# Sudo42b/vision.cpp

Hardware: AMD Instinct MI355X
Metric: images/sec, Depth-Anything-V2-Small 518x518 f16 (higher is better)
Workload: dtype f16

## Files before the change

vision.cpp_amd/csrc/kernels_dconv.hip:

```cpp
#include "vx_common.h"

#include <cmath>
#include <cstdlib>
#include <type_traits>

namespace {

typedef __attribute__((address_space(1))) const void* gptr_t;
typedef __attribute__((address_space(3))) void* lptr_t;

constexpr int TRASH_BLOCKS = 1024;
__device__ __attribute__((aligned(16))) unsigned char g_dconv_trash[TRASH_BLOCKS * 8 * 1024];

constexpr int DCONV_TAB_MAX = 1280;
constexpr int CK = 32;
constexpr int PIXB = CK * 2;
constexpr int NW = 8;

struct tile_grid {
    int ncols, nrows, n_main, n_strip, strip_x0;
    __host__ __device__ tile_grid(int H, int W) {
        const int q = W / 32, rem = W % 32;
        const bool strip = rem > 0 && rem <= 16;
        ncols = q + ((rem > 16) ? 1 : 0);
        nrows = (H + 15) / 16;
        n_main = ncols * nrows;
        n_strip = strip ? (H + 31) / 32 : 0;
        strip_x0 = q * 32;
    }
    __host__ __device__ int total() const { return n_main + n_strip; }
};

__device__ __forceinline__ float relu1(float x) { return __int_as_float(max(__float_as_int(x), 0)); }

template <int COUT, int EPI, bool AR, bool STAMP, int RES = 0, int HSV = (COUT == 32 ? 3 : 2), bool BIL = false, bool ONE = false>
__global__ __launch_bounds__(512) void dconv3x3_kernel(const vx_dconv_args p) {
    static_assert(!ONE || COUT == 32, "single-step tiles: COUT = 32 only");
    constexpr int MT = 2;
    constexpr int HALO_PIX = 18 * 34;
    constexpr int HJ = 5, HALO_INSTR = HJ * NW, HALO_BYTES = HALO_INSTR * 1024;
    constexpr int NI = COUT / 32;
    constexpr int W_BYTES = 9 * COUT * PIXB, W_INSTR = W_BYTES / 1024;
    constexpr int WJ = (W_INSTR + NW - 1) / NW;
    constexpr int HS = HSV;
    constexpr int WSLOTS = RES ? RES : 2;
    static_assert(!RES || COUT == 32, "resident slabs are built for COUT = 32 (the COUT = 64 epilogue stages through slab space)");
    static_assert(!BIL || (COUT == 32 && HSV == 2 && !RES && !AR), "the interpolating loader is built for COUT = 32 with two halo stages");
    constexpr int SRC_PIX = 256, SRC_BYTES = SRC_PIX * PIXB, SJ = SRC_BYTES / 1024 / NW;
    constexpr int SRC_BASE = HS * HALO_BYTES;
    constexpr int W_BASE = HS * HALO_BYTES + (BIL ? 2 * SRC_BYTES : 0);
    constexpr int BIAS_BASE = W_BASE + WSLOTS * W_BYTES;
    constexpr int TAB_BASE = BIAS_BASE + ((COUT * 4 + 15) & ~15);
    static_assert(!BIL || TAB_BASE + (DCONV_TAB_MAX + 4) * 8 <= 160 * 1024, "interpolation tables do not fit");
    constexpr int NCH16 = COUT / 8, PITCH = COUT * 2;
    static_assert(BIAS_BASE + COUT * 4 <= 160 * 1024, "LDS ring too large");
    static_assert(256 * PITCH <= HALO_BYTES && 256 * PITCH <= W_BYTES + (COUT == 32 ? HALO_BYTES : 0), "output staging does not fit a stage");

    extern __shared__ __attribute__((aligned(16))) unsigned char smem[];
    float* const s_bias = reinterpret_cast<float*>(smem + BIAS_BASE);

    const int tid = threadIdx.x, lane = tid & 63;
    const int wave = __builtin_amdgcn_readfirstlane(tid >> 6);
    const int r = lane & 31, h = lane >> 5;
    const int H = p.H, W = p.W;
    const tile_grid tg(H, W);
    const int per_image = tg.total();
    const int total = p.B * per_image;

    int t_cur, t_end, t_step;
    {
        const int id = blockIdx.x, xcd = id & 7;
        const int per = total >> 3, rem = total & 7;
        const int lo = xcd < rem ? xcd * (per + 1) : rem * (per + 1) + (xcd - rem) * per;
        t_end = lo + per + (xcd < rem ? 1 : 0);
        t_step = ((int)gridDim.x - xcd + 7) >> 3;
        t_cur = lo + (id >> 3);
    }
    if (t_cur >= t_end) return;

    if (tid < COUT) s_bias[tid] = p.bias ? p.bias[tid] : 0.0f;

    const int up = p.up2 ? 1 : 0;
    const int Hs = BIL ? p.bil_hs : H >> up, Ws = BIL ? p.bil_ws : W >> up;
    const int nch = p.cin / CK;
    const int nch_total_bytes = nch * 9 * COUT * PIXB;
    const long x_plane_bytes = p.x_plane * 2;
    const int x_pix = p.x_pix ? (int)p.x_pix : CK;
    const long out_pix = p.out_pix ? p.out_pix : CK, res1_pix = p.res1_pix ? p.res1_pix : CK, res2_pix = p.res2_pix ? p.res2_pix : CK;

    uint2* const tab_y = reinterpret_cast<uint2*>(smem + TAB_BASE);
    uint2* const tab_x = tab_y + H + 2;
    if constexpr (BIL) {
        const float sfy = (H > 1 && Hs > 1) ? (float)(H - 1) / (float)(Hs - 1) : (float)H / (float)Hs;
        const float sfx = (W > 1 && Ws > 1) ? (float)(W - 1) / (float)(Ws - 1) : (float)W / (float)Ws;
        for (int i = tid; i < H + W + 4; i += 512) {
            const bool isx = i >= H + 2;
            const int o = (isx ? i - (H + 2) : i) - 1, n_out = isx ? W : H, n_src = isx ? Ws : Hs;
            uint2 e = {0x80000000u, 0u};
            if (o >= 0 && o < n_out) {
                const float sc = (float)o / (isx ? sfx : sfy);
                int i0 = (int)floorf(sc);
                i0 = max(0, min(i0, n_src - 1));
                const float f = fminf(fmaxf(sc - (float)i0, 0.0f), 1.0f);
                e.x = (i0 + 1 < n_src ? 0x40000000u : 0u) | (unsigned)i0 << 16;
                e.y = (unsigned)__builtin_bit_cast(unsigned short, (f16)(1.0f - f)) | (unsigned)__builtin_bit_cast(unsigned short, (f16)f) << 16;
            }
            tab_y[i] = e;
        }
        __syncthreads();
    }

    struct geom { int b, y0, x0, tws; };
    auto locate = [&](int t) {
        geom g;
        g.b = t / per_image;
        const int k = t - g.b * per_image;
        if (k < tg.n_main) {
            const int ty = k / tg.ncols;
            g.y0 = ty * 16; g.x0 = (k - ty * tg.ncols) * 32; g.tws = 5;
        } else {
            g.y0 = (k - tg.n_main) * 32; g.x0 = tg.strip_x0; g.tws = 4;
        }
        return g;
    };
    constexpr unsigned OOB = 0x80000000u;
    unsigned hoff[HJ];
    unsigned hpack[HJ];
    auto setup_shape_src = [&](int tws) {
        const int hw = (1 << tws) + 2;
#pragma unroll
        for (int j = 0; j < HJ; ++j) {
            const int L = (wave + j * NW) * 64 + lane;
            const int pix = L >> 2, phys = L & 3;
            const int hy = tws == 5 ? pix / 34 : pix / 18;
            const int hx = pix - hy * hw;
            hpack[j] = (unsigned)(pix < HALO_PIX ? hy : 255) | (unsigned)hx << 8 | (unsigned)(phys ^ ((pix >> 2) & 3)) << 16 | (pix < HALO_PIX ? 1u << 24 : 0u);
        }
    };
    __amdgpu_buffer_rsrc_t x_rsrc;
    const __amdgpu_buffer_rsrc_t w_rsrc = __builtin_amdgcn_make_buffer_rsrc(const_cast<void*>(p.w), 0, nch_total_bytes, 0x00020000);
    auto setup_src = [&](const geom& g) {
        const long img_bytes = (long)Hs * Ws * x_pix * 2;
        const long span = x_pix > CK ? img_bytes : (nch - 1) * x_plane_bytes + img_bytes;
        x_rsrc = __builtin_amdgcn_make_buffer_rsrc(const_cast<char*>(reinterpret_cast<const char*>(p.x)) + g.b * img_bytes, 0, (int)span, 0x00020000);
#pragma unroll
        for (int j = 0; j < HJ; ++j) {
            unsigned pk = hpack[j];
            asm volatile("" : "+v"(pk));
            const int iy = g.y0 - 1 + (int)(pk & 0xff), ix = g.x0 - 1 + (int)((pk >> 8) & 0xff);
            const bool valid = (pk >> 24) && (unsigned)iy < (unsigned)H && (unsigned)ix < (unsigned)W;
            const int e = ((iy >> up) * Ws + (ix >> up)) * x_pix + (int)(((pk >> 16) & 3) << 3);
            hoff[j] = valid ? (unsigned)(e * 2) : OOB;
        }
    };
    unsigned spack[SJ];
    unsigned soff[SJ];
    auto patch_w = [](int tws) { return tws == 5 ? 21 : 12; };
    auto setup_shape_patch = [&](int tws) {
        const int pw = patch_w(tws);
#pragma unroll
        for (int j = 0; j < SJ; ++j) {
            const int L = (wave + j * NW) * 64 + lane, q = L >> 2;
            const int prow = q / pw;
            spack[j] = (unsigned)prow | (unsigned)(q - prow * pw) << 8 | (unsigned)(L & 3) << 16 | (q < 252 ? 1u << 24 : 0u);
        }
    };
    auto patch_origin = [&](int y0, int x0, int& py0, int& px0) {
        py0 = (__builtin_amdgcn_readfirstlane(tab_y[max(y0 - 1, 0) + 1].x) >> 16) & 0x3fff;
        px0 = (__builtin_amdgcn_readfirstlane(tab_x[max(x0 - 1, 0) + 1].x) >> 16) & 0x3fff;
    };
    auto setup_patch = [&](const geom& g) {
        const long img_bytes = (long)Hs * Ws * x_pix * 2;
        const long span = x_pix > CK ? img_bytes : (nch - 1) * x_plane_bytes + img_bytes;
        x_rsrc = __builtin_amdgcn_make_buffer_rsrc(const_cast<char*>(reinterpret_cast<const char*>(p.x)) + g.b * img_bytes, 0, (int)span, 0x00020000);
        int py0, px0;
        patch_origin(g.y0, g.x0, py0, px0);
#pragma unroll
        for (int j = 0; j < SJ; ++j) {
            unsigned pk = spack[j];
            asm volatile("" : "+v"(pk));
            const int sy = py0 + (int)(pk & 0xff), sx = px0 + (int)((pk >> 8) & 0xff);
            const bool valid = (pk >> 24) && sy < Hs && sx < Ws;
            soff[j] = valid ? (unsigned)(((sy * Ws + sx) * x_pix + (int)(((pk >> 16) & 3) << 3)) * 2) : OOB;
        }
    };
    auto issue_patch = [&](int c, int sstage) {
#pragma unroll
        for (int j = 0; j < SJ; ++j)
            __builtin_amdgcn_raw_ptr_buffer_load_lds(x_rsrc, (lptr_t)(smem + SRC_BASE + sstage * SRC_BYTES + (wave + j * NW) * 1024), 16, soff[j],
                                                     c * (int)x_plane_bytes, 0, 0);
    };
    unsigned ioff[HJ], ifr[HJ];
    unsigned short idy[HJ];
    int i_shape = -1;
    auto setup_interp = [&](const geom& g) {
        if (g.tws != i_shape) {
            i_shape = g.tws;
            setup_shape_src(i_shape);
        }
        int py0, px0;
        patch_origin(g.y0, g.x0, py0, px0);
        const int pw = patch_w(g.tws), org = py0 * pw + px0;
#pragma unroll
        for (int j = 0; j < HJ; ++j) {
            unsigned pk = hpack[j];
            asm volatile("" : "+v"(pk));
            const uint2 ty = tab_y[min(g.y0 + (int)(pk & 0xff), H + 1)], tx = tab_x[min(g.x0 + (int)((pk >> 8) & 0xff), W + 1)];
            const bool outside = (int)(ty.x | tx.x) < 0;
            const int sy = (ty.x >> 16) & 0x3fff, sx = (tx.x >> 16) & 0x3fff;
            const unsigned lg16 = ((pk >> 16) & 3) * 16;
            const unsigned o00 = (outside ? 252u * PIXB : (unsigned)((sy * pw + sx - org) * PIXB)) + lg16;
            ioff[j] = o00 | (o00 + (outside ? 0u : ((tx.x >> 30) & 1) * PIXB)) << 16;
            idy[j] = (unsigned short)(outside ? 0u : ((ty.x >> 30) & 1) * (unsigned)(pw * PIXB));
            ifr[j] = (tx.y >> 16) | (ty.y & 0xffff0000u);
        }
    };
    typedef _Float16 h2 __attribute__((ext_vector_type(2)));
    auto lerp2 = [](h2 v, h2 w, h2 f) { return f * w + (v - f * v); };
    auto interp_unit = [&](int j, int sstage, int hstage) {
        const unsigned char* const sp = smem + SRC_BASE + sstage * SRC_BYTES;
        const unsigned o0 = ioff[j] & 0xffffu, o1 = ioff[j] >> 16, dy = idy[j];
        const f16x8 a = *reinterpret_cast<const f16x8*>(sp + o0), b = *reinterpret_cast<const f16x8*>(sp + o1);
        const f16x8 c = *reinterpret_cast<const f16x8*>(sp + o0 + dy), d = *reinterpret_cast<const f16x8*>(sp + o1 + dy);
        const h2 fr = __builtin_bit_cast(h2, ifr[j]);
        const h2 fx = __builtin_shufflevector(fr, fr, 0, 0), fy = __builtin_shufflevector(fr, fr, 1, 1);
        f16x8 o;
#pragma unroll
        for (int q = 0; q < 4; ++q) {
            const h2 aa = {a[2 * q], a[2 * q + 1]}, bb = {b[2 * q], b[2 * q + 1]}, cc = {c[2 * q], c[2 * q + 1]}, dd = {d[2 * q], d[2 * q + 1]};
            const h2 r = lerp2(lerp2(aa, bb, fx), lerp2(cc, dd, fx), fy);
            o[2 * q] = r[0];
            o[2 * q + 1] = r[1];
        }
        *reinterpret_cast<f16x8*>(smem + hstage * HALO_BYTES + ((wave + j * NW) * 64 + lane) * 16) = o;
    };

    auto halo_piece = [&](int j, int c, int hstage) {
        __builtin_amdgcn_raw_ptr_buffer_load_lds(x_rsrc, (lptr_t)(smem + hstage * HALO_BYTES + (wave + j * NW) * 1024), 16, hoff[j], c * (int)x_plane_bytes, 0, 0);
    };
    const int slab_rot = (int)((blockIdx.x * 5u + (blockIdx.x >> 3) * 3u) % (unsigned)W_INSTR);
    auto slab_piece = [&](int j, int c, int wslot) {
        const int i = wave + j * NW;
        if (i < W_INSTR) {
            int ir = i;
            if constexpr (COUT == 64) {
                ir += slab_rot;
                ir = ir >= W_INSTR ? ir - W_INSTR : ir;
            }
            __builtin_amdgcn_raw_ptr_buffer_load_lds(w_rsrc, (lptr_t)(smem + W_BASE + wslot * W_BYTES + ir * 1024), 16, lane * 16, c * W_BYTES + ir * 1024, 0, 0);
        }
    };
    auto issue_halo = [&](int c, int hstage) {
#pragma unroll
        for (int j = 0; j < HJ; ++j) halo_piece(j, c, hstage);
    };
    auto issue_slab = [&](int c, int wslot) {
#pragma unroll
        for (int j = 0; j < WJ; ++j) slab_piece(j, c, wslot);
    };

    constexpr int NWIN = MT + 2;
    int a_addr[3][NWIN][2];
    auto setup_addr = [&](int tws) {
        const int hw = (1 << tws) + 2;
        const int row0 = tws == 5 ? 2 * wave : 4 * wave + 2 * (r >> 4), col0 = tws == 5 ? r : (r & 15);
#pragma unroll
        for (int u = 0; u < NWIN; ++u)
#pragma unroll
            for (int kx = 0; kx < 3; ++kx) {
                const int pix = (row0 + u) * hw + col0 + kx;
#pragma unroll
                for (int ks = 0; ks < 2; ++ks) a_addr[kx][u][ks] = pix * PIXB + (((ks * 2 + h) ^ ((pix >> 2) & 3)) << 4);
            }
    };
    auto out_row = [&](int tws, int mi) { return tws == 5 ? 2 * wave + mi : 4 * wave + mi + 2 * (r >> 4); };
    auto out_col = [&](int tws) { return tws == 5 ? r : (r & 15); };
    int w_addr[2][2];
#pragma unroll
    for (int st = 0; st < 2; ++st)
#pragma unroll
        for (int ks = 0; ks < 2; ++ks) w_addr[st][ks] = W_BASE + st * W_BYTES + r * PIXB + (((ks * 2 + h) ^ ((r >> 2) & 3)) << 4);

    f32x16 acc[MT][NI];
    f32x16 bias_tile, headw_tile;
    if constexpr (COUT == 32) {
#pragma unroll
        for (int g = 0; g < 4; ++g) {
#pragma unroll
            for (int q = 0; q < 4; ++q) {
                bias_tile[4 * g + q] = p.bias ? p.bias[8 * g + 4 * h + q] : 0.0f;
                if constexpr (EPI == VX_DC_HEAD_F32) headw_tile[4 * g + q] = p.head_w[8 * g + 4 * h + q];
            }
        }
    }

    constexpr int NGRP = 6;
    auto load_group = [&](auto hs_c, auto ws_c, int wslot_off, int grp, f16x8 (&af)[NWIN], f16x8 (&wf)[3][NI]) {
        constexpr int HSt = decltype(hs_c)::value, WSt = decltype(ws_c)::value;
        const int kx = grp >> 1, ks = grp & 1;
#pragma unroll
        for (int ky = 0; ky < 3; ++ky)
#pragma unroll
            for (int ni = 0; ni < NI; ++ni)
                wf[ky][ni] = *reinterpret_cast<const f16x8*>(smem + w_addr[RES ? 0 : WSt][ks] + wslot_off + ((ky * 3 + kx) * COUT + ni * 32) * PIXB);
#pragma unroll
        for (int u = 0; u < NWIN; ++u) af[u] = *reinterpret_cast<const f16x8*>(smem + a_addr[kx][u][ks] + HSt * HALO_BYTES);
    };
    auto relu_frag = [](f16x8& a) {
#pragma unroll
        for (int j = 0; j < 8; ++j) a[j] = a[j] > (f16)0 ? a[j] : (f16)0;
    };
    const bool xres = NI == 2 && p.x_residual != 0;
    const f16 inv_s1 = (f16)(1.0f / p.s1);
    auto compute_win = [&](auto hs_c, auto ws_c, int chunk, auto&& feed) {
        f16x8 af[2][NWIN], wf[2][3][NI];
        const int wslot_off = RES ? chunk * W_BYTES : 0;
        load_group(hs_c, ws_c, wslot_off, 0, af[0], wf[0]);
#pragma unroll
        for (int grp = 0; grp < NGRP; ++grp) {
            if (grp + 1 < NGRP) load_group(hs_c, ws_c, wslot_off, grp + 1, af[(grp + 1) & 1], wf[(grp + 1) & 1]);
            __builtin_amdgcn_sched_barrier(0);
            if constexpr (AR) {
#pragma unroll
                for (int u = 0; u < NWIN; ++u) relu_frag(af[grp & 1][u]);
            }
#pragma unroll
            for (int u = 0; u < NWIN; ++u)
#pragma unroll
                for (int mi = 0; mi < MT; ++mi) {
                    const int ky = u - mi;
                    if (ky < 0 || ky > 2) continue;
#pragma unroll
                    for (int ni = 0; ni < NI; ++ni) {
                        if (ONE && grp == 0 && ky == 0)
                            acc[mi][ni] = __builtin_amdgcn_mfma_f32_32x32x16_f16(wf[grp & 1][ky][ni], af[grp & 1][u], bias_tile, 0, 0, 0);
                        else
                            acc[mi][ni] = __builtin_amdgcn_mfma_f32_32x32x16_f16(wf[grp & 1][ky][ni], af[grp & 1][u], acc[mi][ni], 0, 0, 0);
                    }
                }
            feed(2 * grp);
            feed(2 * grp + 1);
            if constexpr (NI == 2) {
                if ((grp >> 1) == 1 && xres && chunk < 2) {
                    const int ks = grp & 1;
                    f16x8 id;
#pragma unroll
                    for (int j = 0; j < 8; ++j) id[j] = (r == ks * 16 + h * 8 + j) ? inv_s1 : (f16)0;
#pragma unroll
                    for (int mi = 0; mi < MT; ++mi) {
                        if (chunk == 0) acc[mi][0] = __builtin_amdgcn_mfma_f32_32x32x16_f16(id, af[grp & 1][mi + 1], acc[mi][0], 0, 0, 0);
                        else acc[mi][NI - 1] = __builtin_amdgcn_mfma_f32_32x32x16_f16(id, af[grp & 1][mi + 1], acc[mi][NI - 1], 0, 0, 0);
                    }
                }
            }
        }
    };
    constexpr int G = 1;
    auto load_group_tap = [&](auto hs_c, auto ws_c, int grp, f16x8 (&af)[G][MT], f16x8 (&wf)[G][NI]) {
        constexpr int HSt = decltype(hs_c)::value, WSt = decltype(ws_c)::value;
#pragma unroll
        for (int q = 0; q < G; ++q) {
            const int step = grp * G + q, tap = step >> 1, ks = step & 1;
#pragma unroll
            for (int ni = 0; ni < NI; ++ni)
                wf[q][ni] = *reinterpret_cast<const f16x8*>(smem + w_addr[WSt][ks] + (tap * COUT + ni * 32) * PIXB);
#pragma unroll
            for (int mi = 0; mi < MT; ++mi)
                af[q][mi] = *reinterpret_cast<const f16x8*>(smem + a_addr[tap % 3][mi + tap / 3][ks] + HSt * HALO_BYTES);
        }
    };
    auto compute_tap = [&](auto hs_c, auto ws_c, int chunk, auto&& feed) {
        f16x8 af[2][G][MT], wf[2][G][NI];
        load_group_tap(hs_c, ws_c, 0, af[0], wf[0]);
#pragma unroll
        for (int grp = 0; grp < 18 / G; ++grp) {
            if (grp + 1 < 18 / G) load_group_tap(hs_c, ws_c, grp + 1, af[(grp + 1) & 1], wf[(grp + 1) & 1]);
            __builtin_amdgcn_sched_barrier(0);
            if constexpr (AR) {
#pragma unroll
                for (int q = 0; q < G; ++q)
#pragma unroll
                    for (int mi = 0; mi < MT; ++mi) relu_frag(af[grp & 1][q][mi]);
            }
#pragma unroll
            for (int q = 0; q < G; ++q)
#pragma unroll
                for (int mi = 0; mi < MT; ++mi)
#pragma unroll
                    for (int ni = 0; ni < NI; ++ni)
                        acc[mi][ni] = __builtin_amdgcn_mfma_f32_32x32x16_f16(wf[grp & 1][q][ni], af[grp & 1][q][mi], acc[mi][ni], 0, 0, 0);
            feed(grp);
            if constexpr (NI == 2) {
                if ((grp * G) >> 1 == 4 && xres && chunk < 2) {
#pragma unroll
                    for (int q = 0; q < G; ++q) {
                        const int ks = (grp * G + q) & 1;
                        f16x8 id;
#pragma unroll
                        for (int j = 0; j < 8; ++j) id[j] = (r == ks * 16 + h * 8 + j) ? inv_s1 : (f16)0;
#pragma unroll
                        for (int mi = 0; mi < MT; ++mi) {
                            if (chunk == 0) acc[mi][0] = __builtin_amdgcn_mfma_f32_32x32x16_f16(id, af[grp & 1][q][mi], acc[mi][0], 0, 0, 0);
                            else acc[mi][NI - 1] = __builtin_amdgcn_mfma_f32_32x32x16_f16(id, af[grp & 1][q][mi], acc[mi][NI - 1], 0, 0, 0);
                        }
                    }
                }
            }
        }
    };
    auto compute = [&](auto hs_c, auto ws_c, int chunk, auto&& feed) {
        if constexpr (COUT == 32) compute_win(hs_c, ws_c, chunk, feed);
        else compute_tap(hs_c, ws_c, chunk, feed);
    };
    auto stage_swz = [](int ml) { return COUT == 32 ? ((ml ^ (ml >> 2)) & 3) : (ml & 7); };
    auto zero_acc = [&]() {
        if constexpr (ONE) return;
#pragma unroll
        for (int mi = 0; mi < MT; ++mi)
#pragma unroll
            for (int ni = 0; ni < NI; ++ni) {
                if constexpr (COUT == 32) {
                    acc[mi][ni] = bias_tile;
                } else {
#pragma unroll
                    for (int e = 0; e < 16; ++e) acc[mi][ni][e] = 0.0f;
                }
            }
    };

    geom cur = locate(t_cur);
    int shape = cur.tws;
    setup_addr(shape);
    int src_shape = shape;
    if constexpr (BIL) {
        setup_shape_patch(src_shape);
        setup_patch(cur);
    } else {
        setup_shape_src(src_shape);
        setup_src(cur);
    }
    int h_t = t_cur, h_c = 0;
    auto move_cursor = [&]() {
        if (++h_c == nch) {
            h_c = 0;
            h_t += t_step;
            if (h_t < t_end) {
                const geom nx = locate(h_t);
                if constexpr (BIL) {
                    if (nx.tws != src_shape) {
                        src_shape = nx.tws;
                        setup_shape_patch(src_shape);
                    }
                    setup_patch(nx);
                } else {
                    if (nx.tws != src_shape) {
                        src_shape = nx.tws;
                        setup_shape_src(src_shape);
                    }
                    setup_src(nx);
                }
            }
        }
    };
    auto advance_halo = [&](int hstage) -> bool {
        if (h_t >= t_end) return false;
        if constexpr (BIL) issue_patch(h_c, hstage);
        else issue_halo(h_c, hstage);
        move_cursor();
        return true;
    };
    if constexpr (RES) {
        for (int k = 0; k < nch; ++k) issue_slab(k, k);
    } else {
        issue_slab(0, 0);
    }
    bool prev_halo = false;
    if constexpr (BIL) {
        advance_halo(0);
        advance_halo(1);
        setup_interp(cur);
        asm volatile("s_waitcnt vmcnt(0)" ::: "memory");
        __builtin_amdgcn_s_barrier();
        asm volatile("" ::: "memory");
#pragma unroll
        for (int j = 0; j < HJ; ++j) interp_unit(j, 0, 0);
    } else {
#pragma unroll
        for (int k = 0; k < HS - 1; ++k) prev_halo = advance_halo(k);
    }
    if (HS == 2) prev_halo = false;
    zero_acc();
    int c = 0;
    bool stores_in_flight = false;
    unsigned long long ph[6] = {0, 0, 0, 0, 0, 0}, t_prev = 0;
    unsigned n_steps = 0;
    auto stamp = [&](int k) {
        if constexpr (STAMP) {
            const unsigned long long t = __builtin_amdgcn_s_memtime();
            ph[k] += t - t_prev;
            t_prev = t;
        }
    };
    if constexpr (STAMP) t_prev = __builtin_amdgcn_s_memtime();
    f16* const trash = reinterpret_cast<f16*>(g_dconv_trash + ((blockIdx.x % TRASH_BLOCKS) * 8 + wave) * 1024 + lane * 16);

    auto step = [&](auto hs_c, auto ws_c) -> bool {
        constexpr int HSt = decltype(hs_c)::value, WSt = decltype(ws_c)::value;
        {
            const bool st = EPI == VX_DC_F16 && stores_in_flight;
            if (HS == 3 && prev_halo) {
                if (st) asm volatile("s_waitcnt vmcnt(%0)" ::"n"(HJ + NCH16) : "memory");
                else asm volatile("s_waitcnt vmcnt(%0)" ::"n"(HJ) : "memory");
            } else {
                if (st) asm volatile("s_waitcnt vmcnt(%0)" ::"n"(NCH16) : "memory");
                else asm volatile("s_waitcnt vmcnt(0)" ::: "memory");
            }
        }
        stores_in_flight = false;
        stamp(0);
        if constexpr (BIL) asm volatile("s_waitcnt lgkmcnt(0)" ::: "memory");
        __builtin_amdgcn_s_barrier();
        asm volatile("" ::: "memory");
        stamp(1);
        const bool last_chunk = c + 1 == nch;
        const bool do_slab = !RES && (!last_chunk || t_cur + t_step < t_end);
        const int slab_c = last_chunk ? 0 : c + 1;
        const bool do_halo = h_t < t_end;
        const int halo_c = h_c;
        constexpr int HNEXT = (HSt + HS - 1) % HS;
        if constexpr (BIL) {
            if (do_slab) issue_slab(slab_c, WSt ^ 1);
            if (do_halo) {
                issue_patch(halo_c, HSt);
                move_cursor();
            }
            const bool do_interp = !last_chunk || t_cur + t_step < t_end;
            if (do_interp && last_chunk) setup_interp(locate(t_cur + t_step));
            stamp(2);
            compute(hs_c, ws_c, c, [&](int k) {
                if (do_interp && (k & 1) && (k >> 1) < HJ) interp_unit(k >> 1, HSt ^ 1, HSt ^ 1);
            });
        } else if constexpr (COUT == 32) {
            if (do_slab) issue_slab(slab_c, WSt ^ 1);
            if (do_halo) {
                issue_halo(halo_c, HNEXT);
                move_cursor();
            }
            stamp(2);
            compute(hs_c, ws_c, c, [](int) {});
        } else {
            compute(hs_c, ws_c, c, [&](int k) {
                if (k < WJ) {
                    if (do_slab) slab_piece(k, slab_c, WSt ^ 1);
                } else if (k - WJ < HJ) {
                    if (do_halo) halo_piece(k - WJ, halo_c, HNEXT);
                }
            });
        }
        stamp(3);
        if (COUT == 64 && do_halo) move_cursor();
        prev_halo = do_halo;
        stamp(2);
        ++n_steps;
        if (++c < nch) return false;

        constexpr int done = HSt;

        if constexpr (EPI == VX_DC_HEAD_F32) {
#pragma unroll
            for (int mi = 0; mi < MT; ++mi) {
                float part = 0.0f;
#pragma unroll
                for (int g = 0; g < 4; ++g)
#pragma unroll
                    for (int q = 0; q < 4; ++q) part += relu1(acc[mi][0][4 * g + q]) * headw_tile[4 * g + q];
                part += __shfl_xor(part, 32, 64);
                const int oy = cur.y0 + out_row(cur.tws, mi), ox = cur.x0 + out_col(cur.tws);
                if (h == 0 && oy < H && ox < W)
                    reinterpret_cast<float*>(p.out)[((long)cur.b * H + oy) * W + ox] = fmaxf(part + p.head_bias, 0.0f) * p.head_scale;
            }
            asm volatile("s_waitcnt vmcnt(0)" ::: "memory");
            prev_halo = false;
        } else if constexpr (EPI == VX_DC_RGB_F32) {
            if (h == 0) {
#pragma unroll
                for (int mi = 0; mi < MT; ++mi) {
                    const int oy = cur.y0 + out_row(cur.tws, mi), ox = cur.x0 + out_col(cur.tws);
                    if (oy < H && ox < W) {
                        float* o = reinterpret_cast<float*>(p.out) + (((long)cur.b * H + oy) * W + ox) * 3;
                        o[0] = acc[mi][0][0];
                        o[1] = acc[mi][0][1];
                        o[2] = acc[mi][0][2];
                    }
                }
            }
            asm volatile("s_waitcnt vmcnt(0)" ::: "memory");
            prev_halo = false;
        } else {
            asm volatile("" ::: "memory");
            __builtin_amdgcn_s_barrier();
            asm volatile("" ::: "memory");
            unsigned char* st;
            if constexpr (COUT == 32) st = smem + done * HALO_BYTES + wave * 64 * PITCH;
            else st = (wave < 4 ? smem + done * HALO_BYTES : smem + W_BASE + WSt * W_BYTES) + (wave & 3) * 64 * PITCH;
            auto stage_tile = [&](auto act_c) {
                constexpr int ACT = decltype(act_c)::value;
#pragma unroll
                for (int mi = 0; mi < MT; ++mi) {
                    const int ml = mi * 32 + r;
#pragma unroll
                    for (int ni = 0; ni < NI; ++ni)
#pragma unroll
                        for (int g = 0; g < 4; ++g) {
                            const int nl = ni * 32 + 8 * g + 4 * h;
                            float4 bias = {0.f, 0.f, 0.f, 0.f};
                            if constexpr (COUT != 32) bias = *reinterpret_cast<const float4*>(s_bias + nl);
                            float v[4] = {acc[mi][ni][4 * g + 0] + bias.x, acc[mi][ni][4 * g + 1] + bias.y,
                                          acc[mi][ni][4 * g + 2] + bias.z, acc[mi][ni][4 * g + 3] + bias.w};
#pragma unroll
                            for (int j = 0; j < 4; ++j) {
                                if constexpr (ACT == 2) v[j] = relu1(v[j]);
                                else if constexpr (ACT == 1) v[j] = fmaxf(v[j], 0.2f * v[j]);
                            }
                            if (xres) {
#pragma unroll
                                for (int j = 0; j < 4; ++j) v[j] *= p.s1;
                            }
                            f16x4 o = {(f16)v[0], (f16)v[1], (f16)v[2], (f16)v[3]};
                            const int c8 = nl >> 2;
                            const int phys16 = (c8 >> 1) ^ stage_swz(ml);
                            *reinterpret_cast<f16x4*>(st + ml * PITCH + phys16 * 16 + (c8 & 1) * 8) = o;
                        }
                }
            };
            if (p.act == 2) stage_tile(std::integral_constant<int, 2>{});
            else if (p.act == 1) stage_tile(std::integral_constant<int, 1>{});
            else stage_tile(std::integral_constant<int, 0>{});
            const char* const R1 = reinterpret_cast<const char*>(p.res1);
            const char* const R2 = reinterpret_cast<const char*>(p.res2);
            constexpr int ROWS_PER_IT = 64 / NCH16, IT_PER_MT = 32 / ROWS_PER_IT;
            constexpr int NB = 4;
            const int j = lane % NCH16, fr0 = lane / NCH16;
            const int jp = j >> 2, je = (j & 3) * 8;
            const bool wide = cur.tws == 5;
            const int oy_b = cur.y0 + (wide ? 2 * wave : 4 * wave), ox_b = cur.x0 + (wide ? fr0 : (fr0 & 15));
            const int tile0 = (cur.b * H + cur.y0) * W + cur.x0;
            const int base = (cur.b * H + oy_b) * W + ox_b;
            const long off1 = ((long)jp * p.res1_plane + je) * 2, off2 = ((long)jp * p.res2_plane + je) * 2, offo = ((long)jp * p.out_plane + je) * 2;
            const bool unit = p.s1 == 1.0f && p.s2 == 1.0f;
            const int rp1 = (int)res1_pix * 2, rp2 = (int)res2_pix * 2, rpo = (int)out_pix * 2;
            asm volatile("s_waitcnt lgkmcnt(0)" ::: "memory");
            const float s1 = p.s1, s2 = p.s2;
#pragma unroll
            for (int ib = 0; ib < NCH16; ib += NB) {
                int pixel[NB];
                bool ok[NB];
                f16x8 ra[NB], rc[NB], v[NB];
#pragma unroll
                for (int it = 0; it < NB; ++it) {
                    const int t = ib + it, fm = t / IT_PER_MT, dfr = ROWS_PER_IT * (t % IT_PER_MT);
                    const int dy = wide ? fm : fm + 2 * (dfr >> 4), dx = wide ? dfr : (dfr & 15);
                    ok[it] = oy_b + dy < H && ox_b + dx < W;
                    pixel[it] = ok[it] ? base + dy * W + dx : tile0;
                }
                if (R1) {
#pragma unroll
                    for (int it = 0; it < NB; ++it) ra[it] = *reinterpret_cast<const f16x8*>(R1 + off1 + (long)pixel[it] * rp1);
                }
                if (R2) {
#pragma unroll
                    for (int it = 0; it < NB; ++it) rc[it] = *reinterpret_cast<const f16x8*>(R2 + off2 + (long)pixel[it] * rp2);
                }
#pragma unroll
                for (int it = 0; it < NB; ++it) {
                    const int ml = (ib + it) * ROWS_PER_IT + fr0;
                    v[it] = *reinterpret_cast<const f16x8*>(st + ml * PITCH + (j ^ stage_swz(ml)) * 16);
                }
#pragma unroll
                for (int it = 0; it < NB; ++it) {
                    if (unit) {
                        if (R1) v[it] = v[it] + ra[it];
                        if (R2) v[it] = v[it] + rc[it];
                    } else {
                        if (R1) {
#pragma unroll
                            for (int q = 0; q < 8; ++q) v[it][q] = (f16)((float)v[it][q] * s1 + (float)ra[it][q]);
                        }
                        if (R2) {
#pragma unroll
                            for (int q = 0; q < 8; ++q) v[it][q] = (f16)((float)v[it][q] * s2 + (float)rc[it][q]);
                        }
                    }
                    f16* dst = ok[it] ? reinterpret_cast<f16*>(reinterpret_cast<char*>(p.out) + offo + (long)pixel[it] * rpo) : trash;
                    *reinterpret_cast<f16x8*>(dst) = v[it];
                }
            }
            stores_in_flight = true;
        }
        stamp(4);

        t_cur += t_step;
        if (t_cur >= t_end) return true;
        cur = locate(t_cur);
        if (cur.tws != shape) {
            shape = cur.tws;
            setup_addr(shape);
        }
        zero_acc();
        c = 0;
        stamp(5);
        return false;
    };
    using std::integral_constant;
    for (;;) {
        if constexpr (HS == 3) {
            if (step(integral_constant<int, 0>{}, integral_constant<int, 0>{})) break;
            if (step(integral_constant<int, 1>{}, integral_constant<int, 1>{})) break;
            if (step(integral_constant<int, 2>{}, integral_constant<int, 0>{})) break;
            if constexpr (RES) continue;
            if (step(integral_constant<int, 0>{}, integral_constant<int, 1>{})) break;
            if (step(integral_constant<int, 1>{}, integral_constant<int, 0>{})) break;
            if (step(integral_constant<int, 2>{}, integral_constant<int, 1>{})) break;
        } else {
            if (step(integral_constant<int, 0>{}, integral_constant<int, 0>{})) break;
            if (step(integral_constant<int, 1>{}, integral_constant<int, 1>{})) break;
        }
    }
    if constexpr (STAMP) {
        if (tid == 0) {
            unsigned long long* o = reinterpret_cast<unsigned long long*>(p.stamps) + (size_t)blockIdx.x * 8;
#pragma unroll
            for (int k = 0; k < 6; ++k) o[k] = ph[k];
            o[6] = n_steps;
            o[7] = __builtin_amdgcn_s_memtime();
        }
    }
}

int dconv_grid_blocks() {
    static int n_cu = 0;
    if (!n_cu) {
        int dev = 0;
        if (hipGetDevice(&dev) != hipSuccess || hipDeviceGetAttribute(&n_cu, hipDeviceAttributeMultiprocessorCount, dev) != hipSuccess || n_cu <= 0) n_cu = 256;
    }
    return n_cu;
}

template <int COUT, int RES, int HSV, bool BIL = false>
constexpr int dconv_smem_bytes() {
    return HSV * (5 * NW * 1024) + (BIL ? 2 * 256 * PIXB : 0) + (RES ? RES : 2) * 9 * COUT * PIXB + (BIL ? ((COUT * 4 + 15) & ~15) + (DCONV_TAB_MAX + 4) * 8 : COUT * 4);
}

template <int COUT, int EPI, bool AR, bool STAMP, int RES = 0, int HSV = (COUT == 32 ? 3 : 2), bool BIL = false, bool ONE = false>
int prepare_variant() {
    static_assert(dconv_smem_bytes<COUT, RES, HSV, BIL>() <= 160 * 1024, "variant does not fit the LDS");
    VX_CHECK(vx_ensure_dynamic_lds(reinterpret_cast<const void*>(&dconv3x3_kernel<COUT, EPI, AR, STAMP, RES, HSV, BIL, ONE>),
                                   dconv_smem_bytes<COUT, RES, HSV, BIL>()));
    return 1;
}

template <int COUT, int EPI, bool AR, bool STAMP, int RES = 0, int HSV = (COUT == 32 ? 3 : 2), bool BIL = false, bool ONE = false>
int launch_variant(const vx_dconv_args& a, hipStream_t s) {
    constexpr int smem = dconv_smem_bytes<COUT, RES, HSV, BIL>();
    if (!prepare_variant<COUT, EPI, AR, STAMP, RES, HSV, BIL, ONE>()) return 0;
    const long tiles = (long)a.B * tile_grid(a.H, a.W).total();
    int blocks = (int)(tiles < dconv_grid_blocks() ? tiles : dconv_grid_blocks());
    if (tiles > dconv_grid_blocks() && dconv_grid_blocks() % 8 == 0) {
        const long per_xcd = (tiles + 7) / 8, cu_per_xcd = dconv_grid_blocks() / 8;
        const long rounds = (per_xcd + cu_per_xcd - 1) / cu_per_xcd;
        const long blocks_per_xcd = (per_xcd + rounds - 1) / rounds;
        blocks = (int)(8 * blocks_per_xcd);
    }
    hipLaunchKernelGGL((dconv3x3_kernel<COUT, EPI, AR, STAMP, RES, HSV, BIL, ONE>), dim3(blocks), dim3(512), smem, s, a);
    VX_LAUNCH_CHECK();
    return 1;
}

template <int COUT, int EPI>
int launch_dconv(const vx_dconv_args& a, hipStream_t s) {
    if constexpr (COUT == 32 && EPI == VX_DC_HEAD_F32) {
        if (a.cin == 32) return a.bil_hs > 0 ? launch_variant<32, EPI, false, false, 0, 2, true, true>(a, s) : launch_variant<32, EPI, false, false, 0, 3, false, true>(a, s);
    }
    if constexpr (COUT == 32 && (EPI == VX_DC_F16 || EPI == VX_DC_HEAD_F32)) {
        if (a.bil_hs > 0) return launch_variant<32, EPI, false, false, 0, 2, true>(a, s);
    }
    if constexpr (EPI == VX_DC_F16) {
        if (a.a_relu) return launch_variant<COUT, EPI, true, false>(a, s);
        if (a.stamps) return launch_variant<COUT, EPI, false, true>(a, s);
        if constexpr (COUT == 32) {
            static const int res_mode = getenv("VISP_DCONV_RES") ? atoi(getenv("VISP_DCONV_RES")) : -1;
            if (res_mode >= 1 && a.cin == 64) return launch_variant<32, EPI, false, false, 2, 3>(a, s);
            if ((res_mode >= 2 && a.cin <= 128) || (res_mode < 0 && a.cin == 128)) return launch_variant<32, EPI, false, false, 4, 2>(a, s);
        }
    }
    return launch_variant<COUT, EPI, false, false>(a, s);
}


__global__ void esr_tiles_in_kernel(const uint8_t* __restrict__ img, int B, int w, int h, int ch, int ir, int ig, int ib,
                                    vx_tile_layout t, f16* __restrict__ out) {
    const long n = (long)B * t.n_x * t.n_y * t.tile_h * t.tile_w;
    const long i = (long)blockIdx.x * blockDim.x + threadIdx.x;
    if (i >= n) return;
    const int x = (int)(i % t.tile_w);
    long q = i / t.tile_w;
    const int y = (int)(q % t.tile_h);
    q /= t.tile_h;
    const int tile = (int)(q % (t.n_x * t.n_y)), b = (int)(q / (t.n_x * t.n_y));
    const int cx = tile % t.n_x, cy = tile / t.n_x;
    const int sx = min(cx * (t.tile_w - t.overlap_x) + x, w - 1), sy = min(cy * (t.tile_h - t.overlap_y) + y, h - 1);
    const uint8_t* s = img + (((long)b * h + sy) * w + sx) * ch;
    const int idx[3] = {ir, ig, ib};
    f16x8 lo = {0, 0, 0, 0, 0, 0, 0, 0};
#pragma unroll
    for (int c = 0; c < 3; ++c) {
        const float v = (float)s[idx[c]] / 255.0f;
        const f16 hi = (f16)v;
        lo[c] = hi;
        lo[3 + c] = (f16)(v - (float)hi);
    }
    f16x8* o = reinterpret_cast<f16x8*>(out + i * 32);
    const f16x8 z = {0, 0, 0, 0, 0, 0, 0, 0};
    o[0] = lo;
    o[1] = z;
    o[2] = z;
    o[3] = z;
}

__global__ void esr_tiles_in_f32_kernel(const uint8_t* __restrict__ img, int B, int w, int h, int ch, int ir, int ig, int ib, vx_tile_layout t, float* __restrict__ out) {
    const long n = (long)B * t.n_x * t.n_y * t.tile_h * t.tile_w;
    const long i = (long)blockIdx.x * blockDim.x + threadIdx.x;
    if (i >= n) return;
    const int x = (int)(i % t.tile_w);
    long q = i / t.tile_w;
    const int y = (int)(q % t.tile_h);
    q /= t.tile_h;
    const int tile = (int)(q % (t.n_x * t.n_y)), b = (int)(q / (t.n_x * t.n_y));
    const int cx = tile % t.n_x, cy = tile / t.n_x;
    const int sx = min(cx * (t.tile_w - t.overlap_x) + x, w - 1), sy = min(cy * (t.tile_h - t.overlap_y) + y, h - 1);
    const uint8_t* s = img + (((long)b * h + sy) * w + sx) * ch;
    out[i * 3 + 0] = (float)s[ir] / 255.0f;
    out[i * 3 + 1] = (float)s[ig] / 255.0f;
    out[i * 3 + 2] = (float)s[ib] / 255.0f;
}

__device__ __forceinline__ int tl_start(int c, int tile, int overlap, int pad) { return c * (tile - overlap) + (c == 0 ? 0 : pad); }
__device__ __forceinline__ int tl_end(int c, int n, int tile, int overlap, int pad, int image) {
    const int e = c * (tile - overlap) + tile - (c == n - 1 ? 0 : pad);
    return e < image ? e : image;
}

__global__ void esr_tiles_out_kernel(const float* __restrict__ tiles, int B, vx_tile_layout t, float* __restrict__ out_f32,
                                     uint8_t* __restrict__ out_rgba) {
    const long n = (long)B * t.image_h * t.image_w;
    const long i = (long)blockIdx.x * blockDim.x + threadIdx.x;
    if (i >= n) return;
    const int x = (int)(i % t.image_w);
    const int y = (int)((i / t.image_w) % t.image_h);
    const int b = (int)(i / ((long)t.image_w * t.image_h));
    float d[3] = {0.0f, 0.0f, 0.0f};
    {
#pragma clang fp contract(off)
        for (int cy = 0; cy < t.n_y; ++cy) {
            const int by = tl_start(cy, t.tile_h, t.overlap_y, 0), ey = tl_end(cy, t.n_y, t.tile_h, t.overlap_y, 0, t.image_h);
            if (y < by || y >= ey) continue;
            const int pby = tl_start(cy, t.tile_h, t.overlap_y, t.overlap_y), pey = tl_end(cy, t.n_y, t.tile_h, t.overlap_y, t.overlap_y, t.image_h);
            for (int cx = 0; cx < t.n_x; ++cx) {
                const int bx = tl_start(cx, t.tile_w, t.overlap_x, 0), ex = tl_end(cx, t.n_x, t.tile_w, t.overlap_x, 0, t.image_w);
                if (x < bx || x >= ex) continue;
                const int pbx = tl_start(cx, t.tile_w, t.overlap_x, t.overlap_x), pex = tl_end(cx, t.n_x, t.tile_w, t.overlap_x, t.overlap_x, t.image_w);
                float weight = 1.0f;
                int covx = 0, covy = 0;
                if (x < pbx) { weight *= (float)(t.overlap_x - (pbx - x) + 1); covx = t.overlap_x; }
                else if (x >= pex) { weight *= (float)(t.overlap_x - (x - pex)); covx = t.overlap_x; }
                if (y < pby) { weight *= (float)(t.overlap_y - (pby - y) + 1); covy = t.overlap_y; }
                else if (y >= pey) { weight *= (float)(t.overlap_y - (y - pey)); covy = t.overlap_y; }
                const float* tv = tiles + ((((long)b * t.n_y + cy) * t.n_x + cx) * t.tile_h + (y - by)) * (long)t.tile_w * 3 + (long)(x - bx) * 3;
                if (weight > 0.0f) {
                    const float blend = weight / (float)((covx + 1) * (covy + 1));
                    for (int c = 0; c < 3; ++c) d[c] = d[c] + blend * tv[c];
                } else {
                    for (int c = 0; c < 3; ++c) d[c] = tv[c];
                }
            }
        }
    }
    if (out_f32) {
        out_f32[i * 3 + 0] = d[0];
        out_f32[i * 3 + 1] = d[1];
        out_f32[i * 3 + 2] = d[2];
    }
    if (out_rgba) {
        uchar4 o;
        o.x = (uint8_t)(fminf(fmaxf(d[0], 0.0f), 1.0f) * 255.0f);
        o.y = (uint8_t)(fminf(fmaxf(d[1], 0.0f), 1.0f) * 255.0f);
        o.z = (uint8_t)(fminf(fmaxf(d[2], 0.0f), 1.0f) * 255.0f);
        o.w = 255;
        reinterpret_cast<uchar4*>(out_rgba)[i] = o;
    }
}

}

extern "C" int vx_dconv_prepare(void) {
    return prepare_variant<32, VX_DC_F16, false, false>() && prepare_variant<32, VX_DC_F16, true, false>() &&
           prepare_variant<32, VX_DC_F16, false, false, 2, 3>() && prepare_variant<32, VX_DC_F16, false, false, 4, 2>() &&
           prepare_variant<64, VX_DC_F16, false, false>() && prepare_variant<64, VX_DC_F16, true, false>() &&
           prepare_variant<32, VX_DC_RGB_F32, false, false>() && prepare_variant<32, VX_DC_HEAD_F32, false, false>() &&
           prepare_variant<32, VX_DC_F16, false, false, 0, 2, true>() && prepare_variant<32, VX_DC_HEAD_F32, false, false, 0, 2, true>() &&
           prepare_variant<32, VX_DC_HEAD_F32, false, false, 0, 2, true, true>() && prepare_variant<32, VX_DC_HEAD_F32, false, false, 0, 3, false, true>();
}

extern "C" int vx_dconv_bilinear_supported(int cout, int H, int W, int hs, int ws) {
    if (cout != 32 || H < 2 || W < 2 || hs < 2 || ws < 2 || hs > H || ws > W || H + W > DCONV_TAB_MAX) return 0;
    const double ry = (double)(hs - 1) / (double)(H - 1), rx = (double)(ws - 1) / (double)(W - 1);
    auto rows = [](double r, int n) { return (int)std::floor((n - 1) * r + 1.0) + 2; };
    return rows(ry, 18) <= 12 && rows(rx, 34) <= 21 && rows(ry, 34) <= 21 && rows(rx, 18) <= 12;
}

extern "C" int vx_dconv3x3_f16(const vx_dconv_args* args, void* stream) {
    const vx_dconv_args& a = *args;
    VX_REQUIRE(a.x && a.w && a.out, "vx_dconv3x3_f16: null operand");
    VX_REQUIRE(a.cin >= 32 && a.cin % 32 == 0, "vx_dconv3x3_f16: Cin %d must be a multiple of 32", a.cin);
    VX_REQUIRE(a.B > 0 && a.H > 0 && a.W > 0, "vx_dconv3x3_f16: empty extent");
    VX_REQUIRE((int64_t)a.B * a.H * a.W < (int64_t)0x7fffffff && a.out_pix < (1 << 20) && a.res1_pix < (1 << 20) && a.res2_pix < (1 << 20),
               "vx_dconv3x3_f16: pixel indices must fit 32 bits; run fewer images per call");
    VX_REQUIRE(!a.up2 || (a.H % 2 == 0 && a.W % 2 == 0), "vx_dconv3x3_f16: upsampled extent must be even");
    VX_REQUIRE(a.bil_hs <= 0 || (!a.up2 && !a.a_relu && !a.x_residual && !a.stamps && vx_dconv_bilinear_supported(a.cout, a.H, a.W, a.bil_hs, a.bil_ws)),
               "vx_dconv3x3_f16: bilinear input %dx%d -> %dx%d (cout %d) is outside the interpolating loader's limits", a.bil_ws, a.bil_hs, a.W, a.H, a.cout);
    VX_REQUIRE(a.res2_hs <= 0, "vx_dconv3x3_f16: bilinear res2 is not built");
    VX_REQUIRE((reinterpret_cast<uintptr_t>(a.x) & 15) == 0 && (reinterpret_cast<uintptr_t>(a.w) & 15) == 0 &&
               (reinterpret_cast<uintptr_t>(a.out) & 15) == 0, "vx_dconv3x3_f16: operands must be 16-byte aligned");
    {
        const int64_t src_pixels = a.bil_hs > 0 ? (int64_t)a.bil_hs * a.bil_ws : (int64_t)(a.H >> (a.up2 ? 1 : 0)) * (a.W >> (a.up2 ? 1 : 0));
        const int64_t xp = a.x_pix ? a.x_pix : 32;
        VX_REQUIRE(xp >= 32 && xp % 8 == 0 && a.out_pix % 8 == 0 && a.res1_pix % 8 == 0 && a.res2_pix % 8 == 0, "vx_dconv3x3_f16: pixel strides must be multiples of 8 (input >= 32)");
        VX_REQUIRE(a.cin == 32 || (a.x_plane % 8 == 0 && (xp > 32 ? a.x_plane >= 32 : a.x_plane >= (int64_t)a.B * src_pixels * 32)), "vx_dconv3x3_f16: bad input plane stride");
        VX_REQUIRE((int64_t)(a.cin / 32 - 1) * a.x_plane * 2 + src_pixels * xp * 2 < (int64_t)0x7fffffff,
                   "vx_dconv3x3_f16: input planes span more than 2 GiB; run fewer images per call");
    }
    hipStream_t s = as_stream(stream);
    if (a.epi == VX_DC_RGB_F32) {
        VX_REQUIRE(a.cout == 32 && !a.a_relu, "vx_dconv3x3_f16: the rgb head takes weights padded to 32 outputs");
        return launch_dconv<32, VX_DC_RGB_F32>(a, s);
    }
    if (a.epi == VX_DC_HEAD_F32) {
        VX_REQUIRE(a.cout == 32 && a.head_w && !a.a_relu, "vx_dconv3x3_f16: the fused depth head is a 32-channel epilogue with head_w set");
        return launch_dconv<32, VX_DC_HEAD_F32>(a, s);
    }
    VX_REQUIRE(a.epi == VX_DC_F16, "vx_dconv3x3_f16: unknown epilogue %d", a.epi);
    VX_REQUIRE(a.out_plane % 8 == 0 && a.res1_plane % 8 == 0 && a.res2_plane % 8 == 0, "vx_dconv3x3_f16: plane strides must be multiples of 8");
    VX_REQUIRE(!a.x_residual || (a.cout == 64 && a.cin >= 64 && !a.res1 && !a.up2 && a.s1 != 0.0f),
               "vx_dconv3x3_f16: x_residual needs cout = 64 <= cin, no res1, no upsampling");
    if (a.cout == 32) return launch_dconv<32, VX_DC_F16>(a, s);
    if (a.cout == 64) return launch_dconv<64, VX_DC_F16>(a, s);
    vx_set_error("vx_dconv3x3_f16: Cout %d not in {32, 64}", a.cout);
    return 0;
}

extern "C" int vx_esrgan_tiles_in(const uint8_t* img, int B, int w, int h, int format, const vx_tile_layout* t, void* out, void* stream) {
    int ch, ir, ig, ib;
    switch (format) {
        case 0: ch = 4; ir = 0; ig = 1; ib = 2; break;
        case 1: ch = 4; ir = 2; ig = 1; ib = 0; break;
        case 2: ch = 4; ir = 1; ig = 2; ib = 3; break;
        case 3: ch = 3; ir = 0; ig = 1; ib = 2; break;
        default: vx_set_error("vx_esrgan_tiles_in: unsupported image format %d", format); return 0;
    }
    const long n = (long)B * t->n_x * t->n_y * t->tile_h * t->tile_w;
    hipLaunchKernelGGL(esr_tiles_in_kernel, dim3((unsigned)((n + 255) / 256)), dim3(256), 0, as_stream(stream), img, B, w, h, ch, ir, ig, ib, *t,
                       reinterpret_cast<f16*>(out));
    VX_LAUNCH_CHECK();
    return 1;
}

extern "C" int vx_esrgan_tiles_in_f32(const uint8_t* img, int B, int w, int h, int format, const vx_tile_layout* t, float* out, void* stream) {
    int ch, ir, ig, ib;
    switch (format) {
        case 0: ch = 4; ir = 0; ig = 1; ib = 2; break;
        case 1: ch = 4; ir = 2; ig = 1; ib = 0; break;
        case 2: ch = 4; ir = 1; ig = 2; ib = 3; break;
        case 3: ch = 3; ir = 0; ig = 1; ib = 2; break;
        default: vx_set_error("vx_esrgan_tiles_in_f32: unsupported image format %d", format); return 0;
    }
    const long n = (long)B * t->n_x * t->n_y * t->tile_h * t->tile_w;
    hipLaunchKernelGGL(esr_tiles_in_f32_kernel, dim3((unsigned)((n + 255) / 256)), dim3(256), 0, as_stream(stream), img, B, w, h, ch, ir, ig, ib, *t, out);
    VX_LAUNCH_CHECK();
    return 1;
}

extern "C" int vx_esrgan_tiles_out(const float* tiles, int B, const vx_tile_layout* t, float* out_f32, uint8_t* out_rgba, void* stream) {
    const long n = (long)B * t->image_h * t->image_w;
    hipLaunchKernelGGL(esr_tiles_out_kernel, dim3((unsigned)((n + 255) / 256)), dim3(256), 0, as_stream(stream), tiles, B, *t, out_f32, out_rgba);
    VX_LAUNCH_CHECK();
    return 1;
}
```

Baseline: 6490.

## Keep COUT=64 weight slabs resident in LDS for Cin=64 direct convs

Adds a resident-weight variant for the COUT=64, Cin=64 direct 3x3 conv, so both weight slabs stay in LDS and the per-chunk slab streaming is dropped; halo pieces now start at the first feed step. To free LDS, the COUT=64 epilogue no longer stages output through slab space: it stages in two rounds through the finished halo stage. This removes repeated weight loads per tile, at the cost of an extra staging round and barrier-free LDS reuse in the epilogue.

```diff
diff --git a/vision.cpp_amd/csrc/kernels_dconv.hip b/vision.cpp_amd/csrc/kernels_dconv.hip
--- a/vision.cpp_amd/csrc/kernels_dconv.hip
+++ b/vision.cpp_amd/csrc/kernels_dconv.hip
@@ -44,7 +44,7 @@
     constexpr int WJ = (W_INSTR + NW - 1) / NW;
     constexpr int HS = HSV;
     constexpr int WSLOTS = RES ? RES : 2;
-    static_assert(!RES || COUT == 32, "resident slabs are built for COUT = 32 (the COUT = 64 epilogue stages through slab space)");
+    static_assert(!RES || COUT == 32 || (EPI == VX_DC_F16 && HSV == 2 && RES == 2), "COUT = 64 keeps its slabs resident at Cin = 64 only (2 halo stages + 72 KB)");
     static_assert(!BIL || (COUT == 32 && HSV == 2 && !RES && !AR), "the interpolating loader is built for COUT = 32 with two halo stages");
     constexpr int SRC_PIX = 256, SRC_BYTES = SRC_PIX * PIXB, SJ = SRC_BYTES / 1024 / NW;
     constexpr int SRC_BASE = HS * HALO_BYTES;
@@ -54,7 +54,7 @@
     static_assert(!BIL || TAB_BASE + (DCONV_TAB_MAX + 4) * 8 <= 160 * 1024, "interpolation tables do not fit");
     constexpr int NCH16 = COUT / 8, PITCH = COUT * 2;
     static_assert(BIAS_BASE + COUT * 4 <= 160 * 1024, "LDS ring too large");
-    static_assert(256 * PITCH <= HALO_BYTES && 256 * PITCH <= W_BYTES + (COUT == 32 ? HALO_BYTES : 0), "output staging does not fit a stage");
+    static_assert(NW * 32 * MT * PITCH / (COUT == 64 ? MT : 1) <= HALO_BYTES, "output staging does not fit a halo stage");
 
     extern __shared__ __attribute__((aligned(16))) unsigned char smem[];
     float* const s_bias = reinterpret_cast<float*>(smem + BIAS_BASE);
@@ -356,14 +356,14 @@
         }
     };
     constexpr int G = 1;
-    auto load_group_tap = [&](auto hs_c, auto ws_c, int grp, f16x8 (&af)[G][MT], f16x8 (&wf)[G][NI]) {
+    auto load_group_tap = [&](auto hs_c, auto ws_c, int wslot_off, int grp, f16x8 (&af)[G][MT], f16x8 (&wf)[G][NI]) {
         constexpr int HSt = decltype(hs_c)::value, WSt = decltype(ws_c)::value;
 #pragma unroll
         for (int q = 0; q < G; ++q) {
             const int step = grp * G + q, tap = step >> 1, ks = step & 1;
 #pragma unroll
             for (int ni = 0; ni < NI; ++ni)
-                wf[q][ni] = *reinterpret_cast<const f16x8*>(smem + w_addr[WSt][ks] + (tap * COUT + ni * 32) * PIXB);
+                wf[q][ni] = *reinterpret_cast<const f16x8*>(smem + w_addr[RES ? 0 : WSt][ks] + wslot_off + (tap * COUT + ni * 32) * PIXB);
 #pragma unroll
             for (int mi = 0; mi < MT; ++mi)
                 af[q][mi] = *reinterpret_cast<const f16x8*>(smem + a_addr[tap % 3][mi + tap / 3][ks] + HSt * HALO_BYTES);
@@ -371,10 +371,11 @@
     };
     auto compute_tap = [&](auto hs_c, auto ws_c, int chunk, auto&& feed) {
         f16x8 af[2][G][MT], wf[2][G][NI];
-        load_group_tap(hs_c, ws_c, 0, af[0], wf[0]);
+        const int wslot_off = RES ? chunk * W_BYTES : 0;
+        load_group_tap(hs_c, ws_c, wslot_off, 0, af[0], wf[0]);
 #pragma unroll
         for (int grp = 0; grp < 18 / G; ++grp) {
-            if (grp + 1 < 18 / G) load_group_tap(hs_c, ws_c, grp + 1, af[(grp + 1) & 1], wf[(grp + 1) & 1]);
+            if (grp + 1 < 18 / G) load_group_tap(hs_c, ws_c, wslot_off, grp + 1, af[(grp + 1) & 1], wf[(grp + 1) & 1]);
             __builtin_amdgcn_sched_barrier(0);
             if constexpr (AR) {
 #pragma unroll
@@ -549,11 +550,12 @@
             stamp(2);
             compute(hs_c, ws_c, c, [](int) {});
         } else {
+            constexpr int HK0 = RES ? 0 : WJ;
             compute(hs_c, ws_c, c, [&](int k) {
-                if (k < WJ) {
+                if (k < HK0) {
                     if (do_slab) slab_piece(k, slab_c, WSt ^ 1);
-                } else if (k - WJ < HJ) {
-                    if (do_halo) halo_piece(k - WJ, halo_c, HNEXT);
+                } else if (k - HK0 < HJ) {
+                    if (do_halo) halo_piece(k - HK0, halo_c, HNEXT);
                 }
             });
         }
@@ -600,14 +602,13 @@
             asm volatile("" ::: "memory");
             __builtin_amdgcn_s_barrier();
             asm volatile("" ::: "memory");
-            unsigned char* st;
-            if constexpr (COUT == 32) st = smem + done * HALO_BYTES + wave * 64 * PITCH;
-            else st = (wave < 4 ? smem + done * HALO_BYTES : smem + W_BASE + WSt * W_BYTES) + (wave & 3) * 64 * PITCH;
-            auto stage_tile = [&](auto act_c) {
+            constexpr int ROUNDS = COUT == 64 ? MT : 1, MPR = MT / ROUNDS, IPR = NCH16 / ROUNDS;
+            unsigned char* const st = smem + done * HALO_BYTES + wave * (32 * MPR) * PITCH;
+            auto stage_tile = [&](auto act_c, int round) {
                 constexpr int ACT = decltype(act_c)::value;
 #pragma unroll
-                for (int mi = 0; mi < MT; ++mi) {
-                    const int ml = mi * 32 + r;
+                for (int mi = round * MPR; mi < (round + 1) * MPR; ++mi) {
+                    const int ml = (mi - round * MPR) * 32 + r;
 #pragma unroll
                     for (int ni = 0; ni < NI; ++ni)
 #pragma unroll
@@ -633,13 +634,11 @@
                         }
                 }
             };
-            if (p.act == 2) stage_tile(std::integral_constant<int, 2>{});
-            else if (p.act == 1) stage_tile(std::integral_constant<int, 1>{});
-            else stage_tile(std::integral_constant<int, 0>{});
             const char* const R1 = reinterpret_cast<const char*>(p.res1);
             const char* const R2 = reinterpret_cast<const char*>(p.res2);
             constexpr int ROWS_PER_IT = 64 / NCH16, IT_PER_MT = 32 / ROWS_PER_IT;
             constexpr int NB = 4;
+            static_assert(IPR % NB == 0, "a staging round drains in whole batches");
             const int j = lane % NCH16, fr0 = lane / NCH16;
             const int jp = j >> 2, je = (j & 3) * 8;
             const bool wide = cur.tws == 5;
@@ -649,50 +648,56 @@
             const long off1 = ((long)jp * p.res1_plane + je) * 2, off2 = ((long)jp * p.res2_plane + je) * 2, offo = ((long)jp * p.out_plane + je) * 2;
             const bool unit = p.s1 == 1.0f && p.s2 == 1.0f;
             const int rp1 = (int)res1_pix * 2, rp2 = (int)res2_pix * 2, rpo = (int)out_pix * 2;
-            asm volatile("s_waitcnt lgkmcnt(0)" ::: "memory");
             const float s1 = p.s1, s2 = p.s2;
 #pragma unroll
-            for (int ib = 0; ib < NCH16; ib += NB) {
-                int pixel[NB];
-                bool ok[NB];
-                f16x8 ra[NB], rc[NB], v[NB];
-#pragma unroll
-                for (int it = 0; it < NB; ++it) {
-                    const int t = ib + it, fm = t / IT_PER_MT, dfr = ROWS_PER_IT * (t % IT_PER_MT);
-                    const int dy = wide ? fm : fm + 2 * (dfr >> 4), dx = wide ? dfr : (dfr & 15);
-                    ok[it] = oy_b + dy < H && ox_b + dx < W;
-                    pixel[it] = ok[it] ? base + dy * W + dx : tile0;
-                }
-                if (R1) {
-#pragma unroll
-                    for (int it = 0; it < NB; ++it) ra[it] = *reinterpret_cast<const f16x8*>(R1 + off1 + (long)pixel[it] * rp1);
-                }
-                if (R2) {
-#pragma unroll
-                    for (int it = 0; it < NB; ++it) rc[it] = *reinterpret_cast<const f16x8*>(R2 + off2 + (long)pixel[it] * rp2);
-                }
-#pragma unroll
-                for (int it = 0; it < NB; ++it) {
-                    const int ml = (ib + it) * ROWS_PER_IT + fr0;
-                    v[it] = *reinterpret_cast<const f16x8*>(st + ml * PITCH + (j ^ stage_swz(ml)) * 16);
-                }
-#pragma unroll
-                for (int it = 0; it < NB; ++it) {
-                    if (unit) {
-                        if (R1) v[it] = v[it] + ra[it];
-                        if (R2) v[it] = v[it] + rc[it];
-                    } else {
-                        if (R1) {
-#pragma unroll
-                            for (int q = 0; q < 8; ++q) v[it][q] = (f16)((float)v[it][q] * s1 + (float)ra[it][q]);
+            for (int round = 0; round < ROUNDS; ++round) {
+                if (p.act == 2) stage_tile(std::integral_constant<int, 2>{}, round);
+                else if (p.act == 1) stage_tile(std::integral_constant<int, 1>{}, round);
+                else stage_tile(std::integral_constant<int, 0>{}, round);
+                asm volatile("s_waitcnt lgkmcnt(0)" ::: "memory");
+#pragma unroll
+                for (int ib = round * IPR; ib < (round + 1) * IPR; ib += NB) {
+                    int pixel[NB];
+                    bool ok[NB];
+                    f16x8 ra[NB], rc[NB], v[NB];
+#pragma unroll
+                    for (int it = 0; it < NB; ++it) {
+                        const int t = ib + it, fm = t / IT_PER_MT, dfr = ROWS_PER_IT * (t % IT_PER_MT);
+                        const int dy = wide ? fm : fm + 2 * (dfr >> 4), dx = wide ? dfr : (dfr & 15);
+                        ok[it] = oy_b + dy < H && ox_b + dx < W;
+                        pixel[it] = ok[it] ? base + dy * W + dx : tile0;
+                    }
+                    if (R1) {
+#pragma unroll
+                        for (int it = 0; it < NB; ++it) ra[it] = *reinterpret_cast<const f16x8*>(R1 + off1 + (long)pixel[it] * rp1);
+                    }
+                    if (R2) {
+#pragma unroll
+                        for (int it = 0; it < NB; ++it) rc[it] = *reinterpret_cast<const f16x8*>(R2 + off2 + (long)pixel[it] * rp2);
+                    }
+#pragma unroll
+                    for (int it = 0; it < NB; ++it) {
+                        const int ml = (ib + it - round * IPR) * ROWS_PER_IT + fr0;
+                        v[it] = *reinterpret_cast<const f16x8*>(st + ml * PITCH + (j ^ stage_swz(ml)) * 16);
+                    }
+#pragma unroll
+                    for (int it = 0; it < NB; ++it) {
+                        if (unit) {
+                            if (R1) v[it] = v[it] + ra[it];
+                            if (R2) v[it] = v[it] + rc[it];
+                        } else {
+                            if (R1) {
+#pragma unroll
+                                for (int q = 0; q < 8; ++q) v[it][q] = (f16)((float)v[it][q] * s1 + (float)ra[it][q]);
+                            }
+                            if (R2) {
+#pragma unroll
+                                for (int q = 0; q < 8; ++q) v[it][q] = (f16)((float)v[it][q] * s2 + (float)rc[it][q]);
+                            }
                         }
-                        if (R2) {
-#pragma unroll
-                            for (int q = 0; q < 8; ++q) v[it][q] = (f16)((float)v[it][q] * s2 + (float)rc[it][q]);
-                        }
+                        f16* dst = ok[it] ? reinterpret_cast<f16*>(reinterpret_cast<char*>(p.out) + offo + (long)pixel[it] * rpo) : trash;
+                        *reinterpret_cast<f16x8*>(dst) = v[it];
                     }
-                    f16* dst = ok[it] ? reinterpret_cast<f16*>(reinterpret_cast<char*>(p.out) + offo + (long)pixel[it] * rpo) : trash;
-                    *reinterpret_cast<f16x8*>(dst) = v[it];
                 }
             }
             stores_in_flight = true;
@@ -783,6 +788,13 @@
     }
     if constexpr (COUT == 32 && (EPI == VX_DC_F16 || EPI == VX_DC_HEAD_F32)) {
         if (a.bil_hs > 0) return launch_variant<32, EPI, false, false, 0, 2, true>(a, s);
+    }
+    if constexpr (COUT == 64 && EPI == VX_DC_F16) {
+        if (a.cin == 64) {
+            if (a.a_relu) return launch_variant<64, EPI, true, false, 2, 2>(a, s);
+            if (a.stamps) return launch_variant<64, EPI, false, true, 2, 2>(a, s);
+            return launch_variant<64, EPI, false, false, 2, 2>(a, s);
+        }
     }
     if constexpr (EPI == VX_DC_F16) {
         if (a.a_relu) return launch_variant<COUT, EPI, true, false>(a, s);
@@ -906,6 +918,7 @@
     return prepare_variant<32, VX_DC_F16, false, false>() && prepare_variant<32, VX_DC_F16, true, false>() &&
            prepare_variant<32, VX_DC_F16, false, false, 2, 3>() && prepare_variant<32, VX_DC_F16, false, false, 4, 2>() &&
            prepare_variant<64, VX_DC_F16, false, false>() && prepare_variant<64, VX_DC_F16, true, false>() &&
+           prepare_variant<64, VX_DC_F16, false, false, 2, 2>() && prepare_variant<64, VX_DC_F16, true, false, 2, 2>() &&
            prepare_variant<32, VX_DC_RGB_F32, false, false>() && prepare_variant<32, VX_DC_HEAD_F32, false, false>() &&
            prepare_variant<32, VX_DC_F16, false, false, 0, 2, true>() && prepare_variant<32, VX_DC_HEAD_F32, false, false, 0, 2, true>() &&
            prepare_variant<32, VX_DC_HEAD_F32, false, false, 0, 2, true, true>() && prepare_variant<32, VX_DC_HEAD_F32, false, false, 0, 3, false, true>();
```

New measurement: 6497, median of 6. Within noise of the previous version (+0.1%).
